# NVIDIA/DeepLearningExamples

Measured on AMD Instinct MI355X. Metric: training samples/sec, higher is better.
Workload: dtype bf16; 1 GPU; ResNet-50 v1.5 (PyTorch/Classification/ConvNets) synthetic ImageNet 224x224, label smoothing 0.1, SGD momentum 0.875 (BASELINE.json configs[1]); batch_per_gpu=256, global_batch=256, layout=NHWC, hip_graph=False, parallelism=single GPU

## Files before the change

deeplearningexamples_amd/_cabi.py:

```python
import ctypes
import os

import torch

_HERE = os.path.dirname(os.path.abspath(__file__))
LIB_PATH = os.environ.get("DLE_LIB_PATH") or os.path.join(_HERE, "lib", "libdle_mi355x.so")

F32, F16, BF16 = 0, 1, 2
ACT_NONE, ACT_RELU, ACT_GELU, ACT_RELU_BWD, ACT_ADD, ACT_GELU_BWD, ACT_TANH, ACT_TANH_BWD = 0, 1, 2, 3, 4, 5, 6, 7
ACT_ADD_MASKED, ACT_MUL, ACT_GELU_DAUX = 8, 9, 10

_DT = {torch.float32: F32, torch.float16: F16, torch.bfloat16: BF16}

c_void_p, c_int, c_i64, c_float = ctypes.c_void_p, ctypes.c_int, ctypes.c_int64, ctypes.c_float
c_u64 = ctypes.c_uint64

_SIGS = {
    "dle_last_error": (ctypes.c_char_p, []),
    "dle_abi_version": (c_int, []),
    "dle_device_check": (c_int, [c_int, ctypes.c_char_p, c_int]),
    "dle_dot_interact_out_width": (c_int, [c_int, c_int]),
    "dle_dot_interact_fwd": (c_int, [c_void_p, c_void_p, c_int, c_int, c_int, c_int, c_int, c_void_p]),
    "dle_dot_interact_bwd": (c_int, [c_void_p, c_void_p, c_void_p, c_void_p, c_int, c_int, c_int, c_int,
                                     c_int, c_void_p]),
# ... 50 lines not shown
    "dle_conv3x3_affine_launch_count": (c_i64, []),
    "dle_conv2d_grouped_fwd_affine": (c_int, [c_void_p] * 5 + [c_int] * 9 + [c_void_p]),
    "dle_se_gate": (c_int, [c_void_p] * 6 + [c_int] * 5 + [c_void_p]),
    "dle_se_apply": (c_int, [c_void_p] * 4 + [c_i64, c_int, c_int, c_int, c_int, c_void_p]),
    "dle_dwconv2d_act_fwd": (c_int, [c_void_p] * 6 + [c_i64] + [c_int] * 9 + [c_void_p]),
    "dle_dwconv2d_pool_bands": (c_int, [c_int] * 5),
    "dle_se_gate_act": (c_int, [c_void_p, c_int, c_float] + [c_void_p] * 5 + [c_int] * 4 + [c_void_p]),
    "dle_silu_avgpool_fwd": (c_int, [c_void_p, c_void_p, c_int, c_int, c_int, c_int, c_void_p]),
    "dle_ssd_decode_fwd": (c_int, [c_void_p, c_void_p, c_int, c_void_p, c_void_p, c_void_p, c_int, c_int, c_int, c_float, c_float,
                                   c_int, c_void_p]),
    "dle_ssd_nms_fwd": (c_int, [c_void_p] * 5 + [c_int, c_int, c_int, c_float, c_float, c_int, c_void_p]),
    "dle_ssd_select_fwd": (c_int, [c_void_p] * 9 + [c_int] * 5 + [c_void_p]),
    "dle_conv2d_dgrad": (c_int, [c_void_p, c_void_p, c_void_p, c_void_p] + [c_int] * 10 + [c_void_p]),
    "dle_conv2d_wgrad": (c_int, [c_void_p, c_void_p, c_void_p] + [c_int] * 12 + [c_void_p, c_i64, c_void_p]),
    "dle_nchw_to_nhwc": (c_int, [c_void_p, c_void_p, c_i64, c_int, c_i64, c_int, c_int, c_void_p]),
    "dle_gemm_expand_add_up2": (c_int, [c_void_p, c_void_p, c_void_p, c_void_p, c_int, c_int, c_int, c_i64, c_i64, c_i64, c_i64, c_int,
                                        c_int, c_int, c_int, c_void_p]),
    "dle_conv1x1_bnload_groups": (c_int, [c_int, c_int, c_int]),
    "dle_conv1x1_bnload_fwd": (c_int, [c_void_p] * 11 + [c_i64, c_int, c_int, c_int, c_int, c_void_p]),
    "dle_bn_relu_maxpool_fwd": (c_int, [c_void_p] * 8 + [c_int, c_int, c_int, c_int, c_int, c_void_p]),
    "dle_wgrad1x1_workspace": (c_i64, []),
    "dle_wgrad1x1_mode": (c_int, [c_int]),
    "dle_wgrad1x1_workspace_for": (c_i64, [c_int, c_int, c_int]),
    "dle_gemm8_mode": (c_int, [c_int]),
    "dle_gemm8_min_items": (c_int, [c_int]),
    "dle_gemm8_launch_count": (c_i64, []),
    "dle_wgrad1x1_try": (c_int, [c_void_p, c_void_p, c_void_p, c_int, c_int, c_int, c_int, c_int, c_void_p, c_i64, c_void_p]),
    "dle_conv3x3_wgrad_workspace": (c_i64, []),
    "dle_conv3x3_wgrad_mode": (c_int, [c_int]),
    "dle_stem_conv7_groups": (c_int, [c_int, c_int]),
    "dle_stem_conv7_fwd": (c_int, [c_void_p, c_void_p, c_void_p, c_void_p, c_i64, c_int, c_int, c_int, c_int, c_void_p]),
    "dle_stem_conv7_wgrad_workspace": (c_i64, [c_int, c_int]),
    "dle_stem_conv7_wgrad": (c_int, [c_void_p, c_void_p, c_void_p, c_void_p, c_i64, c_int, c_int, c_int, c_int, c_int, c_void_p]),
    "dle_stem_pack_weight": (c_int, [c_void_p, c_void_p, c_int, c_void_p]),
    "dle_bn_workspace_bytes": (c_i64, [c_i64, c_int]),
    "dle_bn_fwd_stats": (c_int, [c_void_p, c_i64, c_int, c_float, c_float, c_void_p, c_void_p, c_void_p, c_void_p,
                                 c_void_p, c_i64, c_int, c_void_p]),
    "dle_conv2d_fwd_colstats": (c_int, [c_void_p, c_void_p, c_void_p] + [c_int] * 10 + [c_void_p, c_i64, c_void_p, c_void_p]),
    "dle_bn_stats_from_partials": (c_int, [c_void_p, c_int, c_i64, c_int, c_float, c_float, c_void_p, c_void_p, c_void_p,
                                           c_void_p, c_void_p, c_i64, c_void_p]),
    "dle_bn_fwd_apply": (c_int, [c_void_p] * 8 + [c_i64, c_int, c_int, c_int, c_void_p]),
    "dle_rccl_available": (c_int, []),
    "dle_rccl_unique_id": (c_int, [c_void_p]),
    "dle_rccl_init": (c_int, [c_void_p, c_int, c_int, c_void_p]),
    "dle_rccl_count": (c_int, [c_void_p]),
    "dle_rccl_destroy": (c_int, [c_void_p]),
# ... 290 lines not shown
```

deeplearningexamples_amd/csrc/gemm8.hip:

```cpp
#include "gemm8_kernel.h"

static int g8_mode_value = -2;
extern "C" int dle_gemm8_mode(int mode) {
  if (g8_mode_value == -2) g8_mode_value = dle_env_int("DLE_GEMM_8PH", 1);
  const int prev = g8_mode_value;
  if (mode >= 0) g8_mode_value = mode;
  return prev;
}

static int g8_min_items_value = -1;
extern "C" int dle_gemm8_min_items(int n) {
  if (g8_min_items_value < 0) g8_min_items_value = dle_env_int("DLE_GEMM_8PH_MIN_ITEMS", 128);
  const int prev = g8_min_items_value;
  if (n >= 0) g8_min_items_value = n;
  return prev;
}
static long long g8_launches = 0;
extern "C" int64_t dle_gemm8_launch_count(void) { return __atomic_load_n(&g8_launches, __ATOMIC_RELAXED); }

#ifdef G8_TIMING
unsigned long long* g8_dbg_ptr = nullptr;
int g8_dbg_items = 0;
#endif
static int g8_launch_epi0(const Gemm8Args* p, int dt, int am, int bm, int grid, hipStream_t stream) {
#define G8_E0(DT) do { if (am == 0 && bm == 0) g8_launch<DT, 0, 0, 0, ACT_NONE>(*p, grid, stream); \
    else if (am == 0) g8_launch<DT, 0, 1, 0, ACT_NONE>(*p, grid, stream); else g8_launch<DT, 1, 1, 0, ACT_NONE>(*p, grid, stream); } while (0)
  if (dt == DLE_F16) G8_E0(DLE_F16); else G8_E0(DLE_BF16);
#undef G8_E0
  return 1;
}

static int g8_try(const void* A, const void* B, void* C, void* aux, const float* bias, const void* src, int M, int N,
                  int K, int64_t lda, int64_t ldb, int64_t ldc, int a_kc, int b_kc, int in_dtype, int out_dtype,
                  int act, int splitk, int accumulate, float alpha, float* ws, float* stats, int stats_sq, hipStream_t stream) {
  if (dle_gemm8_mode(-1) <= 0) return 0;
  if (in_dtype != DLE_F16 && in_dtype != DLE_BF16) return 0;
  if (!a_kc && b_kc) return 0;
  if (M < 256 || N < 256 || K < 2 * BK || (K & 7) != 0 || (N & 7) != 0) return 0;
  if ((K % BK) != 0 && !(a_kc && lda >= K && (!b_kc || ldb >= K))) return 0;
  if (!a_kc && (M & 7) != 0) return 0;
  const bool al = ((((uintptr_t)A) | ((uintptr_t)B) | ((uintptr_t)C) | ((uintptr_t)src) | ((uintptr_t)bias) |
                    ((uintptr_t)ws)) & 15) == 0 && (lda & 7) == 0 && (ldb & 7) == 0 && (ldc & 7) == 0 &&
                  (((uintptr_t)aux) & ((act == ACT_ADD_MASKED || act == ACT_RELU_BITS || act == ACT_RELU_BWD_BITS) ? 1 : 15)) == 0;
  if (!al) return 0;
  const long long a_rows = a_kc ? M : K, b_rows = b_kc ? N : K;
  const long long a_bytes = a_rows * lda * 2, b_bytes = b_rows * ldb * 2;
  if ((a_rows + 256) * lda * 2 >= 0xFFFFFFFFLL || (b_rows + 256) * ldb * 2 >= 0xFFFFFFFFLL) return 0;
  if ((long long)M * ldc * 4 >= 0x7FFFFFFFFFFFLL) return 0;
  if (splitk < 1) splitk = 1;
  const int ktiles = (K + BK - 1) / BK;
  if (splitk > ktiles) return 0;
  int epi;
  if (splitk > 1) {
    if (!ws || out_dtype != DLE_F32 || bias || act != ACT_NONE || aux || stats) return 0;
    epi = 0;
  } else if (act == ACT_RELU_BWD_BITS) {
    if (src || !aux || bias || out_dtype != in_dtype || accumulate || alpha != 1.0f || ldc != N || (N & 15) != 0 || b_kc) return 0;
    if ((long long)(M + 256) * ldc * 2 >= 0xFFFFFFFFLL) return 0;
    if (stats && (M & 255) != 0) return 0;
    epi = 2;
  } else if (act == ACT_RELU_BITS) {
    if (!aux || stats || out_dtype != in_dtype || accumulate || ldc != N || (N & 15) != 0 || !a_kc || !b_kc) return 0;
    if ((long long)(M + 256) * ldc * 2 >= 0xFFFFFFFFLL) return 0;
    epi = 1;
  } else if (act == ACT_RELU_BWD || act == ACT_ADD || act == ACT_ADD_MASKED || act == ACT_MUL || act == ACT_GELU_BWD || act == ACT_TANH_BWD) {
    if (!src || bias || (aux != nullptr) != (act == ACT_ADD_MASKED) || out_dtype != in_dtype || accumulate || alpha != 1.0f) return 0;
    if (act == ACT_ADD_MASKED && (ldc != N || (N & 15) != 0 || b_kc)) return 0;
    if ((long long)(M + 256) * ldc * 2 >= 0xFFFFFFFFLL) return 0;
    if (stats && !(act == ACT_RELU_BWD || act == ACT_MUL)) return 0;
    if (stats && (M & 255) != 0) return 0;
// ... 8 lines not shown
    } else if (out_dtype != in_dtype || accumulate) return 0;
    if (act == ACT_GELU_DAUX && !aux) return 0;
    epi = (bias || act != ACT_NONE || aux) ? 1 : 0;
  } else return 0;
  const int am = a_kc ? 0 : 1, bm = b_kc ? 0 : 1;
  const long long tiles = (long long)((M + 255) / 256) * ((N + 255) / 256);
  const long long nitems = tiles * splitk;
  const int min_items = dle_gemm8_min_items(-1);
  if (nitems < min_items || nitems > (1 << 22) || splitk > 0x7FFF || ktiles > 0xFFFF) return 0;
  const DleDeviceLimits* lim = dle_device_limits();
  if (!lim || lim->lds_per_block < G8_LDS_BYTES) return 0;
  const int ncu = lim->cus;
  Gemm8Args p = {};
  p.A = (const unsigned short*)A; p.B = (const unsigned short*)B; p.C = C; p.aux = aux; p.bias = bias;
  p.src = (const unsigned short*)src; p.ws = splitk > 1 ? ws : nullptr; p.stats = stats;
  p.M = M; p.N = N; p.K = K; p.lda = lda; p.ldb = ldb; p.ldc = ldc;
  p.a_bytes = (unsigned)a_bytes; p.b_bytes = (unsigned)b_bytes;
  p.out_dtype = out_dtype; p.act = act; p.splitk = splitk; p.accumulate = accumulate; p.alpha = alpha;
  p.gm = dle_gemm_gm();
  {
    const long long cb = splitk > 1 ? (long long)M * N * 4 : (long long)M * ldc * (out_dtype == DLE_F32 ? 4 : 2);
    p.c_bytes = cb < 0xFFFFFFFFLL ? (unsigned)cb : 0u;
  }
  p.nitems = (int)nitems;
  p.tiles_m = (M + 255) / 256; p.tiles_n = (N + 255) / 256; p.ktiles = ktiles;
#ifdef G8_TIMING
  p.dbg = g8_dbg_ptr; p.dbg_items = g8_dbg_items;
#endif
  const int grid = (int)(nitems < ncu ? nitems : ncu);
  p.grid = grid;
  if ((nitems + grid - 1) / grid > G8_TBL_ITEMS) return 0;
  int launched;
  if (epi == 3) {
    if (in_dtype == DLE_F16) g8_launch<DLE_F16, 0, 0, 3, ACT_NONE>(p, grid, stream); else g8_launch<DLE_BF16, 0, 0, 3, ACT_NONE>(p, grid, stream);
    launched = 1;
  } else if (epi == 0) launched = g8_launch_epi0(&p, in_dtype, am, bm, grid, stream);
  else if (epi == 1) launched = g8_launch_epi1(&p, in_dtype, am, bm, act, grid, stream);
  else launched = g8_launch_epi2(&p, in_dtype, am, bm, act, grid, stream);
  if (!launched) return 0;
  hipError_t e = hipGetLastError();
  if (e != hipSuccess) { dle_set_error("gemm8 launch failed: %s", hipGetErrorString(e)); return (int)e + 1000; }
  __atomic_fetch_add(&g8_launches, 1, __ATOMIC_RELAXED);
  return 1;
}

extern "C" int dle_gemm8_try(const void* A, const void* B, void* C, void* aux, const float* bias, const void* src, int M, int N,
                             int K, int64_t lda, int64_t ldb, int64_t ldc, int a_kc, int b_kc, int in_dtype, int out_dtype,
                             int act, int splitk, int accumulate, float alpha, float* ws, float* stats, hipStream_t stream) {
  return g8_try(A, B, C, aux, bias, src, M, N, K, lda, ldb, ldc, a_kc, b_kc, in_dtype, out_dtype, act, splitk, accumulate, alpha, ws,
                stats, 0, stream);
}

extern "C" int dle_gemm8_colstats_try(const void* A, const void* B, void* C, int M, int N, int K, int64_t lda, int64_t ldb, int64_t ldc,
                                      int dtype, float* stats, hipStream_t stream) {
  if (!stats) return 0;
  return g8_try(A, B, C, nullptr, nullptr, nullptr, M, N, K, lda, ldb, ldc, 1, 1, dtype, dtype, ACT_NONE, 1, 0, 1.0f, nullptr, stats, 1,
                stream);
}

extern "C" int dle_gemm8_relu_bits_try(const void* X, const void* W, void* Y, void* bits, const float* bias, int M, int N, int K,
                                       int64_t ldx, int64_t ldw, int dtype, hipStream_t stream) {
  return g8_try(X, W, Y, bits, bias, nullptr, M, N, K, ldx, ldw, N, 1, 1, dtype, dtype, ACT_RELU_BITS, 1, 0, 1.0f, nullptr, nullptr, 0,
                stream);
}

extern "C" int dle_gemm8_relu_bwd_bits_try(const void* dY, const void* W, void* dX, const void* bits, float* colsum_partial, int M,
                                           int N, int K, int64_t lddy, int64_t ldw, int dtype, hipStream_t stream) {
  return g8_try(dY, W, dX, (void*)bits, nullptr, nullptr, M, N, K, lddy, ldw, N, 1, 0, dtype, dtype, ACT_RELU_BWD_BITS, 1, 0, 1.0f,
                nullptr, colsum_partial, 0, stream);
}
```

deeplearningexamples_amd/csrc/gemm8_kernel.h:

```cpp
#pragma once
#include "gemm_tiles.h"
#include "gemm8_walk.h"

#define G8_HALF 8192
#define G8_BUF (4 * G8_HALF)
#define G8_STAGE_BYTES (2 * G8_BUF * 2)
#define G8_TS_PITCH 80
#define G8_TS_BYTES (32 * G8_TS_PITCH)
#define G8_TS_BASE (G8_STAGE_BYTES + 8 * 256)
#define G8_TBL_BASE (G8_TS_BASE + 8 * G8_TS_BYTES)
#define G8_TBL_ITEMS 512
#define G8_LDS_BYTES (G8_TBL_BASE + G8_TBL_ITEMS * 16)
#define G8_WAVE_FENCE() __builtin_amdgcn_fence(__ATOMIC_SEQ_CST, "wavefront")

struct Gemm8Args {
  const unsigned short* A;
  const unsigned short* B;
  void* C;
  void* aux;
  const float* bias;
  const unsigned short* src;
  float* ws;
  float* stats;
  int M, N, K;
  long long lda, ldb, ldc;
  unsigned a_bytes, b_bytes;
  int out_dtype, act, splitk, accumulate;
  float alpha;
  int gm;
  unsigned c_bytes;
  int nitems, grid;
  int tiles_m, tiles_n, ktiles;
#ifdef G8_TIMING
  unsigned long long* dbg;
  int dbg_items;
#endif
};
extern "C" int g8_launch_epi1(const Gemm8Args* p, int dt, int am, int bm, int act, int grid, hipStream_t stream);
extern "C" int g8_launch_epi2(const Gemm8Args* p, int dt, int am, int bm, int act, int grid, hipStream_t stream);
#ifdef G8_TIMING
#define G8_STAMP(slot) do { if ((wave & 3) == 0 && lane == 0 && p.dbg && item_seq < p.dbg_items) \
    p.dbg[((((long long)blockIdx.x * 2 + wr) * p.dbg_items) + item_seq) * 4 + (slot)] = __builtin_readcyclecounter(); } while (0)
#else
#define G8_STAMP(slot) do { } while (0)
#endif

#define G8_ST_KEEP 16
#define G8_SB() __builtin_amdgcn_sched_barrier(0)
#define G8_BARRIER() do { G8_SB(); asm volatile("s_barrier" ::: "memory"); G8_SB(); } while (0)
#define G8_LGKM(N) do { G8_SB(); asm volatile("s_waitcnt lgkmcnt(%0)" :: "n"(N) : "memory"); G8_SB(); } while (0)
#define G8_VM(N) do { G8_SB(); asm volatile("s_waitcnt vmcnt(%0)" :: "n"(N) : "memory"); G8_SB(); } while (0)

__device__ __forceinline__ int g8_perm32(int i) { return 16 * ((i >> 2) & 1) + 4 * (i >> 3) + (i & 3); }

template <bool PERM>
// ... 103 lines not shown
  return 0.5f * x * (1.0f + g8_tanh2(k0 * (x + k1 * x * x * x)));
}
__device__ __forceinline__ float2v_t g8_gelu_d2(float2v_t x, float2v_t& d) {
  const float k0 = 0.7978845608028654f, k1 = 0.044715f;
  const float2v_t x2 = x * x;
  const float2v_t th = g8_tanh2(k0 * (x + k1 * x2 * x));
  const float2v_t hp = 0.5f * (1.0f + th);
  d = hp + 0.5f * x * (1.f - th * th) * k0 * (1.f + 3.f * k1 * x2);
  return x * hp;
}
__device__ __forceinline__ float g8_gelu(float x) {
  const float k0 = 0.7978845608028654f, k1 = 0.044715f;
  return 0.5f * x * (1.0f + fast_tanh(k0 * (x + k1 * x * x * x)));
}
__device__ __forceinline__ float g8_gelu_d(float x, float& d) {
  const float k0 = 0.7978845608028654f, k1 = 0.044715f;
  const float x2 = x * x;
  const float th = fast_tanh(k0 * (x + k1 * x2 * x));
  const float hp = 0.5f * (1.0f + th);
  d = hp + 0.5f * x * (1.f - th * th) * k0 * (1.f + 3.f * k1 * x2);
  return x * hp;
}

template <int DT, int AM, int BMD, int EPI, int ACT>
__global__ __launch_bounds__(512, 1) void gemm8_kernel(const Gemm8Args p) {
  extern __shared__ __attribute__((aligned(16))) unsigned char smem_raw[];
  unsigned short* lds = (unsigned short*)smem_raw;
  const int tid = threadIdx.x, lane = tid & 63;
  const int wave = __builtin_amdgcn_readfirstlane(tid >> 6);
  const int wr = wave >> 2, wc = wave & 3;
  constexpr bool RCA = AM == 1, RCB = BMD == 1;
  constexpr int NRA = RCA ? 16 : 8;

  const int G = p.grid;
  const int my_items = __builtin_amdgcn_readfirstlane((p.nitems - (int)blockIdx.x + G - 1) / G);
  int* tbl = (int*)(smem_raw + G8_TBL_BASE);
  for (int i = tid; i < my_items; i += 512) {
    const G8WalkItem w = g8_walk_item((int)blockIdx.x + i * G, p.nitems, p.tiles_m, p.tiles_n, p.ktiles, p.splitk, p.gm);
    *(int4v_t*)(tbl + 4 * i) = (int4v_t){w.m0, w.n0, w.kt0, w.slice_and_tiles};
  }
  __syncthreads();
  auto decode = [&](int li, int& m0, int& n0, int& kt0, int& kt1, int& ky) __attribute__((always_inline)) {
    const int4v_t r = *(const int4v_t*)(tbl + 4 * li);
    m0 = __builtin_amdgcn_readfirstlane(r.x);
    n0 = __builtin_amdgcn_readfirstlane(r.y);
    kt0 = __builtin_amdgcn_readfirstlane(r.z);
    const int w = __builtin_amdgcn_readfirstlane(r.w);
// ... 15 lines not shown
      decode(c_item, c_m0, c_n0, kt0, kt1, ky);
      c_k0 = kt0 * BK;
      c_kend = kt1 * BK;
    } else {
      c_k0 = 0;
      c_kend = 0x7FFFFFFF;
    }
  };
  auto cursor_next = [&]() __attribute__((always_inline)) {
    c_par ^= 1;
    c_k0 += BK;
    if (c_k0 >= c_kend) {
      ++c_item;
      cursor_load();
    }
  };
  const unsigned lds0 = (unsigned)(__UINTPTR_TYPE__)(lds_void*)lds;
  auto stage_piece = [&](auto OPC, auto HFC, auto JC) __attribute__((always_inline)) {
    constexpr int OP = decltype(OPC)::value, HF = decltype(HFC)::value, j = decltype(JC)::value;
    constexpr int MODE = OP == 0 ? AM : BMD;
    const int R0 = (OP == 0 ? c_m0 : c_n0) + HF * 128;
    const int nrows = OP == 0 ? p.M : p.N;
    const unsigned ld = (unsigned)(OP == 0 ? p.lda : p.ldb);
    const unsigned sb = (MODE == 0 ? (unsigned)R0 * ld + (unsigned)c_k0 : (unsigned)c_k0 * ld + (unsigned)R0) * 2u;
    const unsigned total = OP == 0 ? p.a_bytes : p.b_bytes;
    const unsigned nrec = (c_valid && sb < total) ? total - sb : 0u;
    const unsigned long long base = (unsigned long long)(OP == 0 ? p.A : p.B) + sb;
    int4v_t rs;
    rs.x = (int)(unsigned)base;
    rs.y = (int)(unsigned)(base >> 32);
    rs.z = (int)nrec;
    rs.w = 0x00020000;
    const unsigned dst = lds0 + (unsigned)(c_par * G8_BUF + (OP == 0 ? 0 : 2 * G8_HALF) + HF * G8_HALF + wave * 1024) * 2u;
    unsigned vo;
    if constexpr (OP == 0) vo = ((MODE == 0 ? c_k0 + la.c8[j] < p.K : R0 + la.c8[j] < nrows)) ? la.voff[j] : OOB_OFF;
    else vo = ((MODE == 0 ? c_k0 + lb.c8[j] < p.K : R0 + lb.c8[j] < nrows)) ? lb.voff[j] : OOB_OFF;
    g8_dma(rs, dst + j * 1024, vo);
  };
  auto stage = [&](auto OPC, auto HFC) __attribute__((always_inline)) {
    stage_piece(OPC, HFC, std::integral_constant<int, 0>());
    stage_piece(OPC, HFC, std::integral_constant<int, 1>());
  };
  typedef std::integral_constant<int, 0> I0;
  typedef std::integral_constant<int, 1> I1;

  cursor_load();
  stage(I1(), I0()); stage(I0(), I0()); stage(I1(), I1()); stage(I0(), I1());
  cursor_next();
  stage(I1(), I0()); stage(I0(), I0()); stage(I1(), I1()); stage(I0(), I1());
  cursor_next();
  G8_VM(8);
  G8_BARRIER();
  if (wr == 1) G8_BARRIER();

  float16_t acc[2][2][2];
  typename FragT<RCA>::type fa[2][4];
  typename FragT<RCB>::type fb0[4], fb1[4];

// ... 516 lines not shown
          if ((fr & 1) == 0 && col < p.N) {
            if constexpr (EPI == 3) q->stats[(prow * 2 + which) * p.N + col] = a1;
            else q->stats[prow * p.N + col] = a1;
          }
        };
#pragma unroll
        for (int j = 0; j < 2; ++j) {
          reduce_store(st[j], j, 0);
          if constexpr (EPI == 3) reduce_store(st2[j], j, 1);
        }
      }
    }
    if (wr == 1) G8_BARRIER();
#ifdef G8_TIMING
    G8_STAMP(2);
    ++item_seq;
#endif
  }
  if (wr == 0) G8_BARRIER();
  G8_VM(0);
}


template <int DT, int AM, int BMD, int EPI, int ACT>
static void g8_launch(const Gemm8Args& p, int grid, hipStream_t stream) {
  DLE_LAUNCH_LDS((gemm8_kernel<DT, AM, BMD, EPI, ACT>), dim3(grid), dim3(512), G8_LDS_BYTES, stream, p);
}
```

deeplearningexamples_amd/csrc/gemm_dma.hip:

```cpp
#include "gemm_tiles.h"

#define SLAB_MODE(p) ((p).ws != nullptr)
#define GEMM2_LDS_BYTES (2 * (BM * BK + BN * BK) * 2)

struct Gemm2Args {
  const unsigned short* A;
  const unsigned short* B;
  void* C;
  void* aux;
  const float* bias;
  const unsigned short* mask_src;
  int M, N, K;
  long long lda, ldb, ldc;
  int out_dtype, act, splitk, accumulate;
  float alpha;
  float* ws;
  ConvGeom cg;
  int batch_inner, batch_count;
  int unused_pad;
  float* stats;
  int force_small;
  int stats_sums;
  long long row_extra;
  FastDiv row_div;
// ... 1001 lines not shown
  p.out_dtype = dtype; p.act = ACT_NONE; p.splitk = 1; p.accumulate = 0; p.alpha = 1.f;
  p.stats = col_partial; p.force_small = 1;
  p.lda = plain ? C : 0;
  p.cg = make_geom(H, W, C, P, Q, R, S, stride, pad, Ko);
  return launch_gemm(p, dtype, plain ? 0 : 2, 0, 0, stream);
}

extern "C" int dle_conv2d_dgrad(const void* dy, const void* w, void* dx, const void* addend, int N, int H, int W,
                                int C, int Ko, int R, int S, int stride, int pad, int dtype, hipStream_t stream) {
  const int P = (H + 2 * pad - R) / stride + 1, Q = (W + 2 * pad - S) / stride + 1;
  if (int rc = conv_check("conv2d_dgrad", N, H, W, C, Ko, R, S, stride, pad, P, Q, dtype)) return rc;
  DLE_CHECK_ARG(dy && w && dx, "conv2d_dgrad: null pointer");
  if (R == 3 && S == 3 && stride == 1 && pad == 1 && !addend)
    DLE_TRY(dle_conv3x3_try(dy, w, dx, nullptr, 0, N, H, W, C, Ko, 1, dtype, stream), return 0);
  Gemm2Args p = {};
  p.A = (const unsigned short*)dy; p.B = (const unsigned short*)w; p.C = dx;
  p.mask_src = (const unsigned short*)addend;
  p.M = N * H * W; p.N = C; p.K = R * S * Ko; p.lda = 0; p.ldb = 0; p.ldc = C;
  p.out_dtype = dtype; p.act = addend ? ACT_ADD : ACT_NONE; p.splitk = 1; p.accumulate = 0; p.alpha = 1.f;
  p.cg = make_geom(H, W, C, P, Q, R, S, stride, pad, Ko);
  return launch_gemm(p, dtype, 4, 5, 0, stream);
}

extern "C" int dle_conv2d_wgrad(const void* dy, const void* x, float* dw, int N, int H, int W, int C, int Ko, int R,
                                int S, int stride, int pad, int dtype, int splitk, int accumulate, void* workspace,
                                int64_t workspace_bytes, hipStream_t stream) {
  const int P = (H + 2 * pad - R) / stride + 1, Q = (W + 2 * pad - S) / stride + 1;
  if (int rc = conv_check("conv2d_wgrad", N, H, W, C, Ko, R, S, stride, pad, P, Q, dtype)) return rc;
  DLE_CHECK_ARG(dy && x && dw, "conv2d_wgrad: null pointer");
  if (R == 3 && S == 3 && stride == 1 && pad == 1)
    DLE_TRY(dle_conv3x3_wgrad_try(dy, x, dw, N, H, W, C, Ko, dtype, accumulate, workspace, workspace_bytes, stream), return 0);
  Gemm2Args p = {};
  p.A = (const unsigned short*)dy; p.B = (const unsigned short*)x; p.C = dw;
  p.M = Ko; p.N = R * S * C; p.K = N * P * Q; p.lda = Ko; p.ldb = 0; p.ldc = (long long)R * S * C;
  p.out_dtype = DLE_F32; p.act = ACT_NONE; p.accumulate = accumulate; p.alpha = 1.f;
  p.cg = make_geom(H, W, C, P, Q, R, S, stride, pad, Ko);
  const int ktiles = (p.K + BK - 1) / BK;
  if (splitk < 1) splitk = 1;
  if (splitk > ktiles) splitk = ktiles;
  p.splitk = splitk;
  if (splitk > 1) {
    const long long need = (long long)splitk * p.M * p.N * 4;
    if (workspace && workspace_bytes >= need && (((uintptr_t)workspace) & 15) == 0) p.ws = (float*)workspace;
    else if (!accumulate) {
      hipError_t e = hipMemsetAsync(dw, 0, (size_t)p.M * p.N * 4, stream);
      if (e != hipSuccess) { dle_set_error("conv2d_wgrad memset: %s", hipGetErrorString(e)); return (int)e; }
    }
  }
  if (int rc = launch_gemm(p, dtype, 1, 3, 0, stream)) return rc;
  if (p.ws) {
    long long g = (((long long)p.M * p.N + 3) / 4 + 15) / 16;
    if (g > 4096) g = 4096;
    if (!launch_splitk_reduce_shallow((const float*)p.ws, dw, p.M, p.N, p.ldc, splitk, accumulate, stream))
      hipLaunchKernelGGL(splitk_reduce_kernel, dim3((unsigned)g), dim3(256), 0, stream, (const float*)p.ws, dw, p.M, p.N,
                         p.ldc, splitk, accumulate);
    hipError_t e = hipGetLastError();
    if (e != hipSuccess) { dle_set_error("splitk_reduce launch failed: %s", hipGetErrorString(e)); return (int)e; }
  }
  return 0;
}


template <int DT>
__global__ __launch_bounds__(256) void dgrad_s2_pack_kernel(const unsigned short* __restrict__ w, unsigned short* __restrict__ out,
                                                            int Ko, int C) {
  const long long total = 9LL * Ko * C;
  for (long long i = (long long)blockIdx.x * blockDim.x + threadIdx.x; i < total; i += (long long)gridDim.x * blockDim.x) {
    const int c = (int)(i % C);
    const long long t = i / C;
    const int rs = (int)(t % 9), ko = (int)(t / 9);
    const int r = rs / 3, sx = rs - r * 3;
    const int a = r == 1 ? 0 : 1, b = sx == 1 ? 0 : 1;
// ... 66 lines not shown
```

deeplearningexamples_amd/csrc/gemm_family.h:

```cpp
#pragma once
#include "common.h"

#define BM 128
#define BN 128
#define BK 64

enum { ACT_NONE = DLE_ACT_NONE, ACT_RELU = DLE_ACT_RELU, ACT_GELU = DLE_ACT_GELU, ACT_RELU_BWD = DLE_ACT_RELU_BWD,
       ACT_ADD = DLE_ACT_ADD, ACT_GELU_BWD = DLE_ACT_GELU_BWD, ACT_TANH = DLE_ACT_TANH, ACT_TANH_BWD = DLE_ACT_TANH_BWD,
       ACT_ADD_MASKED = DLE_ACT_ADD_MASKED,
       ACT_MUL = DLE_ACT_MUL,
       ACT_GELU_DAUX = DLE_ACT_GELU_DAUX,
       ACT_LAST_PUBLIC = DLE_ACT_GELU_DAUX,
       ACT_RELU_BITS = 11, ACT_RELU_BWD_BITS = 12,
       ACT_ADD_RELU = 13 };

inline bool act_needs_src(int act) {
  return act == ACT_RELU_BWD || act == ACT_ADD || act == ACT_GELU_BWD || act == ACT_TANH_BWD || act == ACT_ADD_MASKED || act == ACT_MUL ||
         act == ACT_ADD_RELU;
}

enum { EX_ACT_NONE = 0, EX_ACT_ADD = 1, EX_ACT_ADD_MASKED = 2 };
inline int expand_act_kind(int act) { return act == ACT_NONE ? EX_ACT_NONE : act == ACT_ADD ? EX_ACT_ADD : EX_ACT_ADD_MASKED; }

inline bool dle_gemm_expand_enabled() { return dle_env_int("DLE_GEMM_EXPAND", 1) != 0; }
// ... 6 lines not shown
__device__ __forceinline__ float gelu_tanh(float x) {
  const float k0 = 0.7978845608028654f, k1 = 0.044715f;
  const float u = k0 * (x + k1 * x * x * x);
  return 0.5f * x * (1.0f + fast_tanh(u));
}
__device__ __forceinline__ float gelu_tanh_d(float x, float& d) {
  const float k0 = 0.7978845608028654f, k1 = 0.044715f;
  const float x2 = x * x;
  const float th = fast_tanh(k0 * (x + k1 * x2 * x));
  const float hp = 0.5f * (1.0f + th);
  d = hp + 0.5f * x * (1.f - th * th) * k0 * (1.f + 3.f * k1 * x2);
  return x * hp;
}

extern "C" {
int dle_gemm_dma_try(const void* A, const void* B, void* C, void* aux, const float* bias, const void* mask_src, int M, int N, int K,
                     int64_t lda, int64_t ldb, int64_t ldc, int a_kc, int b_kc, int in_dtype, int out_dtype, int act, int splitk,
                     int accumulate, float alpha, void* workspace, int64_t workspace_bytes, hipStream_t stream);
int dle_gemm8_try(const void* A, const void* B, void* C, void* aux, const float* bias, const void* src, int M, int N, int K,
                  int64_t lda, int64_t ldb, int64_t ldc, int a_kc, int b_kc, int in_dtype, int out_dtype, int act, int splitk,
                  int accumulate, float alpha, float* ws, float* stats, hipStream_t stream);
int dle_gemm8_colstats_try(const void* A, const void* B, void* C, int M, int N, int K, int64_t lda, int64_t ldb, int64_t ldc,
                           int dtype, float* stats, hipStream_t stream);
int dle_gemm8_relu_bwd_bits_try(const void* dY, const void* W, void* dX, const void* bits, float* colsum_partial, int M, int N,
                                int K, int64_t lddy, int64_t ldw, int dtype, hipStream_t stream);
int dle_gemm_smallm_try(const void* A, const void* B, void* C, const float* bias, const void* src, int M, int N, int K, int64_t lda,
                        int64_t ldb, int64_t ldc, int in_dtype, int out_dtype, int act_add, int accumulate, float alpha,
                        hipStream_t stream);
int dle_gemm_expand_try(const void* A, const void* B, void* C, const void* src, const void* bits, float* stats, int M, int N, int K,
                        int64_t lda, int64_t ldb, int64_t ldc, int b_kc, int in_dtype, int out_dtype, int act, hipStream_t stream);
int dle_gemm_expand_groups(int M, int N, int K);
int dle_conv3x3_try(const void* x, const void* w, void* y, float* stats, long long stats_bytes, int N, int H, int W, int C, int Ko,
                    int dgrad, int dtype, hipStream_t stream);
int dle_conv3x3_tiles(int N, int H, int W);
int dle_conv3x3_affine_try(const void* x, const void* w, void* y, const float* scale, const float* shift, const void* residual, int N,
                           int H, int W, int C, int Ko, int dtype, int relu, hipStream_t stream);
int dle_conv3x3_wgrad_try(const void* dy, const void* x, float* dw, int N, int H, int W, int C, int Ko, int dtype, int accumulate,
                          void* workspace, int64_t workspace_bytes, hipStream_t stream);
}
int gemm_regs_launch(const void* A, const void* B, void* C, void* aux, const float* bias, const void* mask_src, int M, int N, int K,
                     int64_t lda, int64_t ldb, int64_t ldc, int a_kc, int b_kc, int in_dtype, int out_dtype, int act, int splitk,
                     int accumulate, float alpha, hipStream_t stream);
hipError_t wgrad1x1_fold(const float* ws, float* dw, long long total4, int G, int accumulate, hipStream_t stream);
```

deeplearningexamples_amd/functional.py:

```python
import ctypes
import os

import torch

from . import _cabi as C


def dot_interact_out_width(rows, cols):
    return C.lib().dle_dot_interact_out_width(rows, cols)


def dot_interact_fwd(x, force_generic=False):
    C.require_cuda(x)
    if x.dim() != 3:
        raise ValueError("dot_interact: expected [batch, rows, cols], got %s" % (tuple(x.shape),))
    x = x.contiguous()
    b, r, c = x.shape
    out = torch.empty((b, dot_interact_out_width(r, c)), dtype=x.dtype, device=x.device)
    C.annotate(bytes=float(b) * (r * c + out.shape[1]) * x.element_size())
    C.call("dle_dot_interact_fwd", C.ptr(x), C.ptr(out), b, r, c, C.dt(x), int(force_generic), C.stream())
    return out


def dot_interact_bwd(x, upstream, force_generic=False, fuse_mlp_grad=False, grad_out=None, found_inf=None):
# ... 903 lines not shown
                         replayable=not accumulate)
    if rc > 1:
        C.check(rc - 1000 if rc > 1000 else -1, "dle_wgrad1x1_try")
    return rc == 1


def conv2d_wgrad(dy, x, rs, stride=1, pad=0, out=None, accumulate=False, splitk=None):
    C.require_cuda(dy, x, out)
    n, p, q, ko = dy.shape
    n2, h, wd, c = x.shape
    r, s = rs
    if n2 != n or not dy.is_contiguous() or not x.is_contiguous() or (p, q) != _conv_out(h, wd, r, s, stride, pad):
        raise ValueError("conv2d_wgrad: shape mismatch")
    if out is None:
        out = torch.empty((ko, r, s, c), dtype=torch.float32, device=x.device)
        accumulate = False
    m_out, n_out, k = ko, r * s * c, n * p * q
    if splitk is None:
        splitk = pick_splitk(m_out, n_out, k, target_blocks=1024)
    need = splitk * m_out * n_out * 4 if splitk > 1 else 0
    if (r, s, stride, pad) == (3, 3, 1, 1):
        need = max(need, int(C.lib().dle_conv3x3_wgrad_workspace()))
    ws = splitk_workspace(x.device, need) if need else None
    C.annotate(flops=2.0 * n * p * q * ko * r * s * c, tag="wgrad %dx%dx%dx%d k%d %dx%d s%d" % (n, h, wd, c, ko, r, s, stride),
               bytes=float(dy.numel() + x.numel()) * 2 + out.numel() * 4.0)
    C.call("dle_conv2d_wgrad", C.ptr(dy), C.ptr(x), C.ptr(out), n, h, wd, c, ko, r, s, stride, pad, C.dt(x), splitk,
           int(accumulate), C.ptr(ws), ws.numel() * 4 if ws is not None else 0, C.stream())
    return out


def nchw_to_nhwc(x, out_dtype, c_padded=None):
    C.require_cuda(x)
    if x.dtype != torch.float32 or x.dim() != 4 or not x.is_contiguous():
        raise ValueError("nchw_to_nhwc expects a contiguous fp32 NCHW tensor")
    n, c, h, w = x.shape
    cp = c_padded or (c + 7) // 8 * 8
    y = torch.empty((n, h, w, cp), dtype=out_dtype, device=x.device)
    C.call("dle_nchw_to_nhwc", C.ptr(x), C.ptr(y), n, c, h * w, cp, C.dt(y), C.stream())
    return y


def u8_nchw_normalize_nhwc(x, mean, std, out_dtype, c_padded=None):
    C.require_cuda(x, mean, std)
    if x.dtype != torch.uint8 or x.dim() != 4 or not x.is_contiguous():
        raise ValueError("u8_nchw_normalize_nhwc expects a contiguous uint8 NCHW tensor")
    n, c, h, w = x.shape
# ... 1367 lines not shown
```

include/dle_mi355x.h:

```cpp
#ifndef DLE_MI355X_H
#define DLE_MI355X_H
#include <stdint.h>

#ifdef __cplusplus
extern "C" {
#endif

typedef struct ihipStream_t* hipStream_t;

enum { DLE_F32 = 0, DLE_F16 = 1, DLE_BF16 = 2 };
enum { DLE_ACT_NONE = 0, DLE_ACT_RELU = 1, DLE_ACT_GELU = 2, DLE_ACT_RELU_BWD = 3, DLE_ACT_ADD = 4,
       DLE_ACT_GELU_BWD = 5, DLE_ACT_TANH = 6, DLE_ACT_TANH_BWD = 7,
       DLE_ACT_ADD_MASKED = 8,
       DLE_ACT_MUL = 9,
       DLE_ACT_GELU_DAUX = 10   };

const char* dle_last_error(void);
int dle_abi_version(void);
int dle_device_check(int device, char* arch_name, int arch_name_len);

int dle_dot_interact_out_width(int rows, int cols);
int dle_dot_interact_fwd(const void* x, void* out, int batch, int rows, int cols, int dtype,
                         int force_generic, hipStream_t stream);
int dle_dot_interact_bwd(const void* x, const void* upstream, void* grad, void* mlp_grad,
// ... 80 lines not shown
#define DLE_DWCONV_TILE_COLS 16
#define DLE_DWCONV_CHUNK 64
int dle_dwconv2d_act_fwd(const void* x, const void* w, void* y, const float* scale, const float* shift, float* pool,
                         int64_t pool_bytes, int N, int H, int W, int C, int ksize, int stride, int in_act, int out_act,
                         int dtype, hipStream_t stream);
int dle_dwconv2d_pool_bands(int H, int W, int C, int ksize, int stride);
#define DLE_SE_GATE_ACT_MAX_C_PLUS_S 16384
int dle_se_gate_act(const float* pool, int G, float inv_hw, const float* w1, const float* b1, const float* w2,
                    const float* b2, float* gate, int N, int C, int S, int act, hipStream_t stream);
int dle_silu_avgpool_fwd(const void* x, void* y, int N, int HW, int C, int dtype, hipStream_t stream);
#define DLE_SSD_MAX_MAPS 8
#define DLE_SSD_MAX_KEEP 256
#define DLE_SSD_MAX_BOXES 16384
int dle_ssd_decode_fwd(const void* const* heads, const int* geom, int nmaps, const float* dboxes_xywh, float* boxes, float* probs,
                       int N, int B, int L, float scale_xy, float scale_wh, int dtype, hipStream_t stream);
int dle_ssd_nms_fwd(const float* boxes, const float* probs, int* kept_idx, float* kept_score, int* kept_count, int N, int B, int L,
                    float threshold, float criteria, int max_num, hipStream_t stream);
int dle_ssd_select_fwd(const float* boxes, const int* kept_idx, const float* kept_score, const int* kept_count, float* det_boxes,
                       int* det_label, float* det_score, int* det_idx, int* det_count, int N, int B, int L, int max_num,
                       int max_output, hipStream_t stream);
int dle_conv2d_wgrad(const void* dy, const void* x, float* dw, int N, int H, int W, int C, int Ko, int R, int S,
                     int stride, int pad, int dtype, int splitk, int accumulate, void* workspace,
                     int64_t workspace_bytes, hipStream_t stream);
int64_t dle_wgrad1x1_workspace(void);
int dle_wgrad1x1_mode(int mode);
int64_t dle_wgrad1x1_workspace_for(int M, int Ko, int C);
int dle_wgrad1x1_try(const void* dy, const void* x, float* dw, int M, int Ko, int C, int dtype, int accumulate, void* workspace,
                     int64_t workspace_bytes, hipStream_t stream);
int64_t dle_conv3x3_wgrad_workspace(void);
int dle_conv3x3_wgrad_mode(int mode);

int dle_colsum(const void* x, float* out, int64_t M, int N, int64_t ld, int dtype, int accumulate,
               void* workspace, int64_t workspace_bytes, hipStream_t stream);
int64_t dle_colsum_batched_workspace_bytes(int n, int64_t M, int N);
int dle_colsum_batched(const int64_t* table_dev, int n, int64_t M, int N, int64_t ld, int dtype, void* workspace,
                       int64_t workspace_bytes, hipStream_t stream);

int64_t dle_mt_table_len(int n_tensors, int n_lists);
int64_t dle_mt_table_fill(int64_t* table_host, int n_tensors, int n_lists, const int64_t* sizes,
                          const void* const* ptrs, int chunk);
int dle_mt_l2norm(const int64_t* table_dev, int n_tensors, int64_t total_chunks, int chunk, int dtype,
                  float* partial_scratch, float* ret, float* ret_per_tensor, int per_tensor,
                  int* noop_flag, hipStream_t stream);
int dle_mt_lamb_stage1(const int64_t* table_dev, int n_tensors, int64_t total_chunks, int chunk,
                       int grad_dtype, const int* noop_flag, float beta1, float beta2, float beta3,
                       const int* step_dev, int bias_correction, float eps, int mode,
// ... 357 lines not shown
```

Before: 13150 samples/s.

## Route strided 1x1 downsample conv wgrad through gemm8 with strided row-map B addressing

Adds a row-map mode to the gemm8 kernel so the B operand's K rows can be addressed with strided pixel offsets computed by fast division. The 1x1 stride-2 downsample convolution weight gradient is then computed straight from the unstrided NHWC input through the faster 8-phase GEMM, in place of the generic GEMM path. It adds a new template instantiation and per-load index arithmetic, and can be turned off with an environment variable. Only the few downsample layers in ResNet-50 are affected.

```diff
diff --git a/deeplearningexamples_amd/_cabi.py b/deeplearningexamples_amd/_cabi.py
--- a/deeplearningexamples_amd/_cabi.py
+++ b/deeplearningexamples_amd/_cabi.py
@@ -96,6 +96,7 @@
     "dle_wgrad1x1_workspace": (c_i64, []),
     "dle_wgrad1x1_mode": (c_int, [c_int]),
     "dle_wgrad1x1_workspace_for": (c_i64, [c_int, c_int, c_int]),
+    "dle_conv_ds_gemm8": (c_int, [c_int]),
     "dle_gemm8_mode": (c_int, [c_int]),
     "dle_gemm8_min_items": (c_int, [c_int]),
     "dle_gemm8_launch_count": (c_i64, []),
diff --git a/deeplearningexamples_amd/csrc/gemm8.hip b/deeplearningexamples_amd/csrc/gemm8.hip
--- a/deeplearningexamples_amd/csrc/gemm8.hip
+++ b/deeplearningexamples_amd/csrc/gemm8.hip
@@ -22,7 +22,11 @@
 unsigned long long* g8_dbg_ptr = nullptr;
 int g8_dbg_items = 0;
 #endif
-static int g8_launch_epi0(const Gemm8Args* p, int dt, int am, int bm, int grid, hipStream_t stream) {
+static int g8_launch_epi0(const Gemm8Args* p, int dt, int am, int bm, int bmap, int grid, hipStream_t stream) {
+  if (bmap) {
+    if (dt == DLE_F16) g8_launch<DLE_F16, 1, 1, 0, ACT_NONE, 1>(*p, grid, stream); else g8_launch<DLE_BF16, 1, 1, 0, ACT_NONE, 1>(*p, grid, stream);
+    return 1;
+  }
 #define G8_E0(DT) do { if (am == 0 && bm == 0) g8_launch<DT, 0, 0, 0, ACT_NONE>(*p, grid, stream); \
     else if (am == 0) g8_launch<DT, 0, 1, 0, ACT_NONE>(*p, grid, stream); else g8_launch<DT, 1, 1, 0, ACT_NONE>(*p, grid, stream); } while (0)
   if (dt == DLE_F16) G8_E0(DLE_F16); else G8_E0(DLE_BF16);
@@ -30,22 +34,34 @@
   return 1;
 }
 
+struct G8RowMap { int div1, div2; long long ext1, ext2, elems; };
+
 static int g8_try(const void* A, const void* B, void* C, void* aux, const float* bias, const void* src, int M, int N,
                   int K, int64_t lda, int64_t ldb, int64_t ldc, int a_kc, int b_kc, int in_dtype, int out_dtype,
-                  int act, int splitk, int accumulate, float alpha, float* ws, float* stats, int stats_sq, hipStream_t stream) {
+                  int act, int splitk, int accumulate, float alpha, float* ws, float* stats, int stats_sq, hipStream_t stream,
+                  const G8RowMap* bmap = nullptr) {
   if (dle_gemm8_mode(-1) <= 0) return 0;
   if (in_dtype != DLE_F16 && in_dtype != DLE_BF16) return 0;
   if (!a_kc && b_kc) return 0;
+  if (bmap) {
+    if (a_kc || b_kc || M < 8 || N < 8 || K < 1 || (M & 7) != 0 || (N & 7) != 0) return 0;
+    if (bmap->div1 < 1 || bmap->div2 < 1 || bmap->ext1 < 0 || ((bmap->ext1 | bmap->ext2) & 7) != 0 || bmap->elems <= 0) return 0;
+    const long long klast = (long long)((K + BK - 1) / BK) * BK - 1;
+    const long long last = klast * ldb + (klast / bmap->div1) * bmap->ext1 + (klast / bmap->div2) * bmap->ext2;
+    if (last < 0 || (last + N + 256) * 2 >= 0xFFFFFF00LL || bmap->elems * 2 >= 0xFFFFFF00LL) return 0;
+    if (stats || bias || aux || src || act != ACT_NONE) return 0;
+  } else {
   if (M < 256 || N < 256 || K < 2 * BK || (K & 7) != 0 || (N & 7) != 0) return 0;
   if ((K % BK) != 0 && !(a_kc && lda >= K && (!b_kc || ldb >= K))) return 0;
+  }
   if (!a_kc && (M & 7) != 0) return 0;
   const bool al = ((((uintptr_t)A) | ((uintptr_t)B) | ((uintptr_t)C) | ((uintptr_t)src) | ((uintptr_t)bias) |
                     ((uintptr_t)ws)) & 15) == 0 && (lda & 7) == 0 && (ldb & 7) == 0 && (ldc & 7) == 0 &&
                   (((uintptr_t)aux) & ((act == ACT_ADD_MASKED || act == ACT_RELU_BITS || act == ACT_RELU_BWD_BITS) ? 1 : 15)) == 0;
   if (!al) return 0;
   const long long a_rows = a_kc ? M : K, b_rows = b_kc ? N : K;
-  const long long a_bytes = a_rows * lda * 2, b_bytes = b_rows * ldb * 2;
-  if ((a_rows + 256) * lda * 2 >= 0xFFFFFFFFLL || (b_rows + 256) * ldb * 2 >= 0xFFFFFFFFLL) return 0;
+  const long long a_bytes = a_rows * lda * 2, b_bytes = bmap ? bmap->elems * 2 : b_rows * ldb * 2;
+  if ((a_rows + 256) * lda * 2 >= 0xFFFFFFFFLL || (!bmap && (b_rows + 256) * ldb * 2 >= 0xFFFFFFFFLL)) return 0;
   if ((long long)M * ldc * 4 >= 0x7FFFFFFFFFFFLL) return 0;
   if (splitk < 1) splitk = 1;
   const int ktiles = (K + BK - 1) / BK;
@@ -100,6 +116,10 @@
     const long long cb = splitk > 1 ? (long long)M * N * 4 : (long long)M * ldc * (out_dtype == DLE_F32 ? 4 : 2);
     p.c_bytes = cb < 0xFFFFFFFFLL ? (unsigned)cb : 0u;
   }
+  if (bmap) {
+    p.b_ext1 = (unsigned)bmap->ext1; p.b_ext2 = (unsigned)bmap->ext2;
+    p.b_div1 = make_fastdiv(bmap->div1); p.b_div2 = make_fastdiv(bmap->div2);
+  }
   p.nitems = (int)nitems;
   p.tiles_m = (M + 255) / 256; p.tiles_n = (N + 255) / 256; p.ktiles = ktiles;
 #ifdef G8_TIMING
@@ -112,7 +132,8 @@
   if (epi == 3) {
     if (in_dtype == DLE_F16) g8_launch<DLE_F16, 0, 0, 3, ACT_NONE>(p, grid, stream); else g8_launch<DLE_BF16, 0, 0, 3, ACT_NONE>(p, grid, stream);
     launched = 1;
-  } else if (epi == 0) launched = g8_launch_epi0(&p, in_dtype, am, bm, grid, stream);
+  } else if (bmap && epi != 0) return 0;
+  else if (epi == 0) launched = g8_launch_epi0(&p, in_dtype, am, bm, bmap != nullptr, grid, stream);
   else if (epi == 1) launched = g8_launch_epi1(&p, in_dtype, am, bm, act, grid, stream);
   else launched = g8_launch_epi2(&p, in_dtype, am, bm, act, grid, stream);
   if (!launched) return 0;
@@ -127,6 +148,19 @@
                              int act, int splitk, int accumulate, float alpha, float* ws, float* stats, hipStream_t stream) {
   return g8_try(A, B, C, aux, bias, src, M, N, K, lda, ldb, ldc, a_kc, b_kc, in_dtype, out_dtype, act, splitk, accumulate, alpha, ws,
                 stats, 0, stream);
+}
+
+extern "C" int dle_gemm8_wgrad_s_try(const void* dy, const void* x, float* dw, int N, int H, int W, int C, int Ko, int P, int Q,
+                                     int stride, int dtype, int splitk, int accumulate, float* ws, hipStream_t stream) {
+  if ((C & 63) != 0 || (Ko & 63) != 0 || stride < 2) return 0;
+  const long long pixels = (long long)N * P * Q;
+  if (pixels >= 0x7FFFFFFFLL - BK) return 0;
+  G8RowMap map;
+  map.div1 = Q; map.ext1 = ((long long)stride * W - (long long)stride * Q) * C;
+  map.div2 = P * Q; map.ext2 = ((long long)H * W - (long long)stride * W * P) * C;
+  map.elems = (long long)N * H * W * C;
+  return g8_try(dy, x, dw, nullptr, nullptr, nullptr, Ko, C, (int)pixels, Ko, (long long)stride * C, C, 0, 0, dtype, DLE_F32, ACT_NONE,
+                splitk, accumulate, 1.0f, ws, nullptr, 0, stream, &map);
 }
 
 extern "C" int dle_gemm8_colstats_try(const void* A, const void* B, void* C, int M, int N, int K, int64_t lda, int64_t ldb, int64_t ldc,
diff --git a/deeplearningexamples_amd/csrc/gemm8_kernel.h b/deeplearningexamples_amd/csrc/gemm8_kernel.h
--- a/deeplearningexamples_amd/csrc/gemm8_kernel.h
+++ b/deeplearningexamples_amd/csrc/gemm8_kernel.h
@@ -31,6 +31,8 @@
   unsigned c_bytes;
   int nitems, grid;
   int tiles_m, tiles_n, ktiles;
+  unsigned b_ext1, b_ext2;
+  FastDiv b_div1, b_div2;
 #ifdef G8_TIMING
   unsigned long long* dbg;
   int dbg_items;
@@ -180,7 +182,7 @@
   return x * hp;
 }
 
-template <int DT, int AM, int BMD, int EPI, int ACT>
+template <int DT, int AM, int BMD, int EPI, int ACT, int BMAP = 0>
 __global__ __launch_bounds__(512, 1) void gemm8_kernel(const Gemm8Args p) {
   extern __shared__ __attribute__((aligned(16))) unsigned char smem_raw[];
   unsigned short* lds = (unsigned short*)smem_raw;
@@ -242,7 +244,9 @@
     const int R0 = (OP == 0 ? c_m0 : c_n0) + HF * 128;
     const int nrows = OP == 0 ? p.M : p.N;
     const unsigned ld = (unsigned)(OP == 0 ? p.lda : p.ldb);
-    const unsigned sb = (MODE == 0 ? (unsigned)R0 * ld + (unsigned)c_k0 : (unsigned)c_k0 * ld + (unsigned)R0) * 2u;
+    constexpr bool MAPPED = OP == 1 && BMAP != 0;
+    static_assert(!BMAP || BMD == 1, "the row map addresses the K rows of a row-contiguous B operand");
+    const unsigned sb = MAPPED ? 0u : (MODE == 0 ? (unsigned)R0 * ld + (unsigned)c_k0 : (unsigned)c_k0 * ld + (unsigned)R0) * 2u;
     const unsigned total = OP == 0 ? p.a_bytes : p.b_bytes;
     const unsigned nrec = (c_valid && sb < total) ? total - sb : 0u;
     const unsigned long long base = (unsigned long long)(OP == 0 ? p.A : p.B) + sb;
@@ -253,7 +257,12 @@
     rs.w = 0x00020000;
     const unsigned dst = lds0 + (unsigned)(c_par * G8_BUF + (OP == 0 ? 0 : 2 * G8_HALF) + HF * G8_HALF + wave * 1024) * 2u;
     unsigned vo;
-    if constexpr (OP == 0) vo = ((MODE == 0 ? c_k0 + la.c8[j] < p.K : R0 + la.c8[j] < nrows)) ? la.voff[j] : OOB_OFF;
+    if constexpr (MAPPED) {
+      const int k = c_k0 + (wave * 2 + j) * 4 + (lane >> 4);
+      const unsigned off = (unsigned)k * ld + (unsigned)fd_div(k, p.b_div1) * p.b_ext1 + (unsigned)fd_div(k, p.b_div2) * p.b_ext2 +
+                           (unsigned)(R0 + lb.c8[j]);
+      vo = (k < p.K && R0 + lb.c8[j] < nrows) ? off * 2u : OOB_OFF;
+    } else if constexpr (OP == 0) vo = ((MODE == 0 ? c_k0 + la.c8[j] < p.K : R0 + la.c8[j] < nrows)) ? la.voff[j] : OOB_OFF;
     else vo = ((MODE == 0 ? c_k0 + lb.c8[j] < p.K : R0 + lb.c8[j] < nrows)) ? lb.voff[j] : OOB_OFF;
     g8_dma(rs, dst + j * 1024, vo);
   };
@@ -816,7 +825,7 @@
 }
 
 
-template <int DT, int AM, int BMD, int EPI, int ACT>
+template <int DT, int AM, int BMD, int EPI, int ACT, int BMAP = 0>
 static void g8_launch(const Gemm8Args& p, int grid, hipStream_t stream) {
-  DLE_LAUNCH_LDS((gemm8_kernel<DT, AM, BMD, EPI, ACT>), dim3(grid), dim3(512), G8_LDS_BYTES, stream, p);
-}
+  DLE_LAUNCH_LDS((gemm8_kernel<DT, AM, BMD, EPI, ACT, BMAP>), dim3(grid), dim3(512), G8_LDS_BYTES, stream, p);
+}
diff --git a/deeplearningexamples_amd/csrc/gemm_dma.hip b/deeplearningexamples_amd/csrc/gemm_dma.hip
--- a/deeplearningexamples_amd/csrc/gemm_dma.hip
+++ b/deeplearningexamples_amd/csrc/gemm_dma.hip
@@ -1047,6 +1047,13 @@
   return launch_gemm(p, dtype, 4, 5, 0, stream);
 }
 
+static int conv_ds_gemm8_value = 1;
+extern "C" int dle_conv_ds_gemm8(int mode) {
+  const int prev = conv_ds_gemm8_value;
+  if (mode >= 0) conv_ds_gemm8_value = mode;
+  return prev;
+}
+
 extern "C" int dle_conv2d_wgrad(const void* dy, const void* x, float* dw, int N, int H, int W, int C, int Ko, int R,
                                 int S, int stride, int pad, int dtype, int splitk, int accumulate, void* workspace,
                                 int64_t workspace_bytes, hipStream_t stream) {
@@ -1072,7 +1079,12 @@
       if (e != hipSuccess) { dle_set_error("conv2d_wgrad memset: %s", hipGetErrorString(e)); return (int)e; }
     }
   }
-  if (int rc = launch_gemm(p, dtype, 1, 3, 0, stream)) return rc;
+  bool launched = false;
+  if (R == 1 && S == 1 && stride > 1 && pad == 0 && conv_ds_gemm8_value != 0 && (splitk == 1 || p.ws))
+    DLE_TRY(dle_gemm8_wgrad_s_try(dy, x, dw, N, H, W, C, Ko, P, Q, stride, dtype, splitk, accumulate, p.ws, stream), launched = true);
+  if (!launched) {
+    if (int rc = launch_gemm(p, dtype, 1, 3, 0, stream)) return rc;
+  }
   if (p.ws) {
     long long g = (((long long)p.M * p.N + 3) / 4 + 15) / 16;
     if (g > 4096) g = 4096;
diff --git a/deeplearningexamples_amd/csrc/gemm_family.h b/deeplearningexamples_amd/csrc/gemm_family.h
--- a/deeplearningexamples_amd/csrc/gemm_family.h
+++ b/deeplearningexamples_amd/csrc/gemm_family.h
@@ -52,6 +52,8 @@
                   int accumulate, float alpha, float* ws, float* stats, hipStream_t stream);
 int dle_gemm8_colstats_try(const void* A, const void* B, void* C, int M, int N, int K, int64_t lda, int64_t ldb, int64_t ldc,
                            int dtype, float* stats, hipStream_t stream);
+int dle_gemm8_wgrad_s_try(const void* dy, const void* x, float* dw, int N, int H, int W, int C, int Ko, int P, int Q, int stride,
+                          int dtype, int splitk, int accumulate, float* ws, hipStream_t stream);
 int dle_gemm8_relu_bwd_bits_try(const void* dY, const void* W, void* dX, const void* bits, float* colsum_partial, int M, int N,
                                 int K, int64_t lddy, int64_t ldw, int dtype, hipStream_t stream);
 int dle_gemm_smallm_try(const void* A, const void* B, void* C, const float* bias, const void* src, int M, int N, int K, int64_t lda,
diff --git a/deeplearningexamples_amd/functional.py b/deeplearningexamples_amd/functional.py
--- a/deeplearningexamples_amd/functional.py
+++ b/deeplearningexamples_amd/functional.py
@@ -949,6 +949,8 @@
     if (r, s, stride, pad) == (3, 3, 1, 1):
         need = max(need, int(C.lib().dle_conv3x3_wgrad_workspace()))
     ws = splitk_workspace(x.device, need) if need else None
+    if (r, s, pad) == (1, 1, 0) and stride > 1:
+        C.lib().dle_conv_ds_gemm8(0 if os.environ.get("DLE_RN50_DS_GEMM8", "1") == "0" else 1)
     C.annotate(flops=2.0 * n * p * q * ko * r * s * c, tag="wgrad %dx%dx%dx%d k%d %dx%d s%d" % (n, h, wd, c, ko, r, s, stride),
                bytes=float(dy.numel() + x.numel()) * 2 + out.numel() * 4.0)
     C.call("dle_conv2d_wgrad", C.ptr(dy), C.ptr(x), C.ptr(out), n, h, wd, c, ko, r, s, stride, pad, C.dt(x), splitk,
diff --git a/include/dle_mi355x.h b/include/dle_mi355x.h
--- a/include/dle_mi355x.h
+++ b/include/dle_mi355x.h
@@ -126,6 +126,7 @@
 int dle_conv2d_wgrad(const void* dy, const void* x, float* dw, int N, int H, int W, int C, int Ko, int R, int S,
                      int stride, int pad, int dtype, int splitk, int accumulate, void* workspace,
                      int64_t workspace_bytes, hipStream_t stream);
+int dle_conv_ds_gemm8(int mode);
 int64_t dle_wgrad1x1_workspace(void);
 int dle_wgrad1x1_mode(int mode);
 int64_t dle_wgrad1x1_workspace_for(int M, int Ko, int C);
```

New measurement: 13170 samples/s, median of 6. No clear change (+0.2%).
